# levje/TrackToLearn

Hardware: AMD Instinct MI355X
Metric: streamline-steps/s at n_actor=262144 (higher is better)
Workload: dtype f32

## Files before the change

include/ttl_hip.h:

```cpp
#ifndef TTL_HIP_H
#define TTL_HIP_H

#include <stddef.h>
#include <stdint.h>

#ifdef __cplusplus
extern "C" {
#endif

#if defined(__GNUC__) || defined(__clang__)
#define TTL_API __attribute__((visibility("default")))
#else
#define TTL_API
#endif

#define TTL_ABI_VERSION 13

#define TTL_OK 0
#define TTL_ERR_INVALID (-1)
#define TTL_ERR_HIP (-2)
#define TTL_ERR_STATE (-3)
#define TTL_ERR_UNSUPPORTED (-4)

#define TTL_MODE_F32 0
// ... 97 lines not shown

TTL_API int ttl_env_harvest_wait(ttl_env *env, const float *state_in, float *state_out,
                         int64_t state_pitch, void *hip_stream,
                         int32_t *n_continue_out);

TTL_API int ttl_env_freerun_begin(ttl_env *env, int32_t *host_counts, void *hip_stream);
TTL_API int ttl_env_freerun_step(ttl_env *env, const float *actions, int32_t n_rows,
                         float *state_out, int64_t state_pitch, double *reward_out,
                         uint8_t *done_out, void *hip_stream);
TTL_API int ttl_env_freerun_end(ttl_env *env, int32_t *n_active_out, int32_t *length_out,
                        int32_t *steps_out, void *hip_stream);
TTL_API int ttl_env_freerun_scripted_actions(ttl_env *env, const float *state, int64_t state_pitch,
                                     int32_t dir_offset, int32_t n_rows, uint32_t seed,
                                     float wobble, float *actions_out, void *hip_stream);

TTL_API int ttl_env_stopping_flags(ttl_env *env, const float *tail, int32_t n,
                           int32_t n_points, uint8_t *flags_out,
                           void *hip_stream);

TTL_API int ttl_env_set_processing_order(ttl_env *env, const int32_t *order, int32_t n,
                                 void *hip_stream);

TTL_API int ttl_env_refresh_processing_order(ttl_env *env, void *hip_stream);

TTL_API int ttl_env_view(ttl_env *env, const int32_t **continue_idx,
                 const int32_t **row_dest, int32_t *length);

#define TTL_PROFILE_CLASSES 4
TTL_API int ttl_env_profile_begin(ttl_env *env, int32_t max_launches,
                          int32_t class_mask );
TTL_API int ttl_env_profile_end(ttl_env *env, double *total_ms ,
                        int32_t *n_launches );

TTL_API int ttl_scripted_actions(const float *state, int64_t state_pitch,
                         int32_t dir_offset, const int32_t *continue_idx,
                         int32_t n, uint32_t seed, uint32_t step, float wobble,
                         float *actions_out, void *hip_stream);

TTL_API int ttl_peaks_from_sh(const float *sh, int64_t n_voxels, int32_t n_coef,
                      const float *sf_matrix, const float *vertices,
                      const int32_t *neighbours, int32_t n_vertices, int32_t degree,
                      int32_t npeaks, float relative_threshold, float absolute_threshold,
                      float min_separation_cos, int32_t max_candidates, float *peaks_out,
                      void *hip_stream);

TTL_API int ttl_oracle_net_forward(const float *dirs, int64_t n, const void *packed_half,
// ... 51 lines not shown
```

tracktolearn_amd/_lib.py:

```python
import ctypes as C
import os

import torch

_PKG = os.path.dirname(os.path.abspath(__file__))
LIB_PATH = os.path.join(_PKG, 'libttl_hip.so')

ABI_VERSION = 13
SH_LINEAR, SH_BRICK4 = 0, 1
MODE_F32 = 0
MODE_F64DIR = 1
MODE_F32NORM = 2
ORDER_ACTIVE = 0
ORDER_PARTITION = 1
ORDER_BY_POSITION = C.c_void_p(1)
ERR_INVALID, ERR_HIP, ERR_STATE, ERR_UNSUPPORTED = -1, -2, -3, -4


class TTLError(RuntimeError):
    pass


class EnvDesc(C.Structure):
    _fields_ = [
# ... 74 lines not shown
                                             C.c_void_p, C.c_void_p]),
    'ttl_tract_coverage': (C.c_int, [C.c_void_p, C.c_void_p, C.c_int32, C.c_void_p, C.c_float,
                                     C.POINTER(C.c_int32), C.c_void_p, C.c_void_p]),
    'ttl_oracle_bonus': (C.c_int, [C.c_void_p, C.c_int32, C.c_void_p, C.c_int32, C.c_double,
                                   C.c_int32, C.c_void_p, C.c_void_p, C.c_void_p]),
    'ttl_env_harvest_wait': (C.c_int, [C.c_void_p, C.c_void_p, C.c_void_p, C.c_int64,
                                       C.c_void_p, C.POINTER(C.c_int32)]),
    'ttl_env_harvest': (C.c_int, [C.c_void_p, C.c_void_p, C.c_void_p,
                                  C.c_int64, C.c_void_p]),
    'ttl_env_freerun_begin': (C.c_int, [C.c_void_p, C.c_void_p, C.c_void_p]),
    'ttl_env_freerun_step': (C.c_int, [C.c_void_p, C.c_void_p, C.c_int32, C.c_void_p,
                                       C.c_int64, C.c_void_p, C.c_void_p, C.c_void_p]),
    'ttl_env_freerun_scripted_actions': (C.c_int, [C.c_void_p, C.c_void_p, C.c_int64,
                                                   C.c_int32, C.c_int32, C.c_uint32,
                                                   C.c_float, C.c_void_p, C.c_void_p]),
    'ttl_env_freerun_end': (C.c_int, [C.c_void_p, C.POINTER(C.c_int32),
                                      C.POINTER(C.c_int32), C.POINTER(C.c_int32),
                                      C.c_void_p]),
    'ttl_env_stopping_flags': (C.c_int, [C.c_void_p, C.c_void_p, C.c_int32,
                                         C.c_int32, C.c_void_p, C.c_void_p]),
    'ttl_env_set_processing_order': (C.c_int, [C.c_void_p, C.c_void_p, C.c_int32,
                                               C.c_void_p]),
    'ttl_env_refresh_processing_order': (C.c_int, [C.c_void_p, C.c_void_p]),
    'ttl_env_view': (C.c_int, [C.c_void_p, C.POINTER(C.c_void_p),
                               C.POINTER(C.c_void_p), C.POINTER(C.c_int32)]),
    'ttl_env_profile_begin': (C.c_int, [C.c_void_p, C.c_int32, C.c_int32]),
    'ttl_env_profile_end': (C.c_int, [C.c_void_p, C.POINTER(C.c_double),
                                      C.POINTER(C.c_int32)]),
    'ttl_scripted_actions': (C.c_int, [C.c_void_p, C.c_int64, C.c_int32,
                                       C.c_void_p, C.c_int32, C.c_uint32,
                                       C.c_uint32, C.c_float, C.c_void_p,
                                       C.c_void_p]),
    'ttl_peaks_from_sh': (C.c_int, [C.c_void_p, C.c_int64, C.c_int32, C.c_void_p,
                                    C.c_void_p, C.c_void_p, C.c_int32, C.c_int32,
                                    C.c_int32, C.c_float, C.c_float, C.c_float,
                                    C.c_int32, C.c_void_p, C.c_void_p]),
    'ttl_resample_streamlines': (C.c_int, [C.c_void_p, C.c_int64, C.c_void_p,
                                           C.c_void_p, C.c_int32, C.c_int32,
                                           C.c_int32, C.c_void_p, C.c_void_p]),
    'ttl_oracle_net_forward': (C.c_int, [C.c_void_p, C.c_int64, C.c_void_p, C.c_void_p,
                                         C.c_void_p, C.c_void_p, C.c_void_p, C.c_void_p,
                                         C.c_int32, C.c_int32, C.c_int32, C.c_void_p,
                                         C.c_void_p]),
    'ttl_pack_streamlines': (C.c_int, [C.c_void_p, C.c_int64, C.c_void_p, C.c_void_p,
                                       C.c_int32, C.c_void_p, C.c_void_p]),
    'ttl_tract_mask_words': (C.c_int32, [C.c_int64]),
# ... 107 lines not shown
```

tracktolearn_amd/csrc/ttl_hip.hip:

```cpp
#include <hip/hip_runtime.h>

#include <atomic>
#include <chrono>
#include <cmath>
#include <cstdarg>
#include <cstdio>
#include <cstdlib>
#include <cstring>
#include <new>

#include "ttl_hip.h"

#include "ttl_internal.h"

#include <map>
#include <mutex>

namespace {
thread_local char g_err[512] = "";
}

int ttl_detail_fail(int code, const char *fmt, ...) {
    va_list ap;
    va_start(ap, fmt);
// ... 521 lines not shown
    if (active) rank = s_rank[threadIdx.x];
    if (active) {
        const size_t o = (size_t)blockIdx.x * BLOCK + rank;
        *reinterpret_cast<float4 *>(P.slot_head + 4 * o) = hd;
        P.slot_dest[o] = pd.y;
    }
    if (active) s_pos[rank] = pd.x;
    __syncthreads();
    const int pos = s_pos[threadIdx.x];
    const bool keep = pos >= 0;
    const unsigned long long mk = __ballot(keep);
    const int below = __popcll(mk & ((1ull << lane) - 1ull));
    if (lane == 0) red[wave] = __popcll(mk);
    __syncthreads();
    int wave_before = 0;
#pragma unroll
    for (int w = 0; w < BLOCK / 64; ++w)
        if (w < wave) wave_before += red[w];
    if (keep) proc_next[before + wave_before + below] = pos;
}

constexpr int TTL_TAIL_MAX_BLOCKS = 4096;

__global__ __launch_bounds__(BLOCK) void k_tail(
    EnvParams P, const int *__restrict__ idx, int *__restrict__ idx_next,
    const int *__restrict__ proc, int *__restrict__ proc_next, int n_active, int n_slots,
    int nb_rows, int order, int n_pts, int *__restrict__ host_word, int seq, int local_sort) {
    __shared__ int s_scan[TTL_TAIL_MAX_BLOCKS];
    __shared__ int s_wave[BLOCK / 64];
    __shared__ unsigned s_key[BLOCK];
    __shared__ int s_pos[BLOCK];
    __shared__ int s_rank[BLOCK];
    const int tid = threadIdx.x, lane = tid & 63, wave = tid >> 6;
    const int per = (nb_rows + BLOCK - 1) / BLOCK;
    const int lo = tid * per;
    int sum = 0;
    for (int k = 0; k < per; ++k)
        if (lo + k < nb_rows) sum += P.block_counts[lo + k];
    int incl = sum;
#pragma unroll
    for (int off = 1; off < 64; off <<= 1) {
        const int v = __shfl_up(incl, off);
        if (lane >= off) incl += v;
    }
    if (lane == 63) s_wave[wave] = incl;
    __syncthreads();
    int run = incl - sum, total = 0;
#pragma unroll
    for (int w = 0; w < BLOCK / 64; ++w) {
        if (w < wave) run += s_wave[w];
        total += s_wave[w];
    }
    for (int k = 0; k < per; ++k)
        if (lo + k < nb_rows) {
            s_scan[lo + k] = run;
// ... 25 lines not shown
    }
    const int j = i;
    const int row = j < n_slots ? proc[j] : -1;
    const bool live = row >= 0;
    float4 hd = float4{0.f, 0.f, 0.f, 0.f};
    int dest = -1, next = -1;
    if (live) {
        const bool stop = P.stop[row] != 0;
        const int pos = s_scan[row / BLOCK] + P.rank[row];
        dest = row;
        if (order == TTL_ORDER_PARTITION) dest = stop ? total + (row - pos) : pos;
        next = stop ? -1 : pos;
        hd = *reinterpret_cast<const float4 *>(P.head + 4 * (size_t)row);
    }
    if (!local_sort) {
        if (j < n_slots) {
            *reinterpret_cast<float4 *>(P.slot_head + 4 * (size_t)j) = hd;
            P.slot_dest[j] = dest;
            proc_next[j] = next;
        }
        return;
    }
    unsigned key = 0xFFFFFFFFu;
    if (live) {
        const unsigned vx = (unsigned)(int)fminf(fmaxf(floorf(hd.x), 0.0f), 1023.0f);
        const unsigned vy = (unsigned)(int)fminf(fmaxf(floorf(hd.y), 0.0f), 1023.0f);
        const unsigned vz = (unsigned)(int)fminf(fmaxf(floorf(hd.z), 0.0f), 1023.0f);
        const unsigned coarse = (((vx >> 6) & 3u) << 4) | (((vy >> 6) & 3u) << 2) | ((vz >> 6) & 3u);
        const unsigned m = (spread3(vx) << 2) | (spread3(vy) << 1) | spread3(vz);
        key = (min(coarse << 18 | m, 0xFFFFFEu) << 8) | (unsigned)tid;
    }
    unsigned sk = key;
#pragma unroll
    for (int size = 2; size <= 64; size <<= 1) {
#pragma unroll
        for (int stride = size >> 1; stride > 0; stride >>= 1) {
            const unsigned other = (unsigned)__shfl_xor((int)sk, stride);
            const bool up = (lane & size) == 0;
            const bool low = (lane & stride) == 0;
            const unsigned mn = min(sk, other), mx = max(sk, other);
            sk = (up == low) ? mn : mx;
        }
    }
    s_key[tid] = sk;
    s_pos[tid] = -1;
    const int n_live = __syncthreads_count(live);
    int srank = lane;
#pragma unroll
    for (int w = 0; w < BLOCK / 64; ++w) {
        if (w == wave) continue;
        const unsigned *srun = s_key + 64 * w;
        int c = 0;
#pragma unroll
        for (int step = 32; step > 0; step >>= 1)
            if (srun[c + step - 1] < sk) c += step;
        if (c == 63 && srun[63] < sk) c = 64;
        srank += c;
    }
    if (sk != 0xFFFFFFFFu) s_rank[sk & 255u] = srank;
    __syncthreads();
    const size_t base = (size_t)blockIdx.x * BLOCK;
    if (live) {
        const int rank = s_rank[tid];
        *reinterpret_cast<float4 *>(P.slot_head + 4 * (base + rank)) = hd;
        P.slot_dest[base + rank] = dest;
        s_pos[rank] = next;
    }
    __syncthreads();
    if (j < n_slots) {
        if (tid >= n_live) P.slot_dest[j] = -1;
        proc_next[j] = s_pos[tid];
    }
}

__global__ __launch_bounds__(BLOCK) void k_probe_flags(
    EnvParams P, const float *__restrict__ tail, int n, int n_pts,
    uint8_t *__restrict__ out) {
    const int i = blockIdx.x * BLOCK + threadIdx.x;
    if (i >= n) return;
    const float *t = tail + (size_t)i * 9;
    float ux, uy, uz, wx, wy, wz;
    int bits;
    if (n_pts >= 2) {
        bits = stopping_bits(P, t[0], t[1], t[2], t[3], t[4], t[5], t[6], t[7],
                             t[8], n_pts, ux, uy, uz, wx, wy, wz);
    } else {
        bits = (n_pts >= P.max_nb_steps) ? TTL_FLAG_LENGTH : 0;
        if (outside_mask(P, t[6], t[7], t[8])) bits |= TTL_FLAG_MASK;
    }
    out[i] = (uint8_t)bits;
}

__global__ __launch_bounds__(BLOCK) void k_finish(EnvParams P,
                                                  const int *__restrict__ idx,
                                                  int n_active, int n_pts) {
// ... 171 lines not shown

inline size_t align_up(size_t v, size_t a) { return (v + a - 1) / a * a; }

}

struct ttl_env {
    ttl_env_desc d;
    EnvParams P;
    int length;
    int n_active;
    int cur;
    int stepped;
    int last_order;
    int last_n;
    uint8_t *last_done;
    int *proc[2];
    char *order_ws;
    size_t order_ws_bytes;
    int proc_cur;
    int use_proc;
    int n_slots;
    int tail_fused;
    int tail_fused_max;
    int state_kernel;
    hipStream_t side;
    hipEvent_t ev_prefix;
    hipEvent_t ev_counts;
    int counts_pending;
    const int32_t *host_counts;
    const int32_t *host_probe;
    int *host_dev;
    int poll_seq;
    hipStream_t poll_stream;
    int fuse_small;
    int poll_counts;
    int local_sort;
    int n_exact;
    int fr_cap;
    int *fr_host_word;
    int prof_on;
    int prof_mask;
    int prof_cap;
    int prof_n[TTL_PROFILE_CLASSES];
    hipEvent_t *prof_ev[TTL_PROFILE_CLASSES];
};

// ... 16 lines not shown
    if (stop) e->prof_n[which]++;
}

extern "C" {

const char *ttl_last_error(void) { return g_err; }
uint32_t ttl_abi_version(void) { return TTL_ABI_VERSION; }
size_t ttl_env_desc_size(void) { return sizeof(ttl_env_desc); }

size_t ttl_env_workspace_bytes(int32_t n_max) {
    if (n_max < 0) return 0;
    const size_t n = (size_t)n_max;
    const size_t nb = (n + BLOCK - 1) / BLOCK + 1;
    size_t b = 0;
    b += align_up(n, 256);
    b += 6 * align_up(n * sizeof(int), 256);
    b += 2 * align_up(n * 4 * sizeof(float), 256);
    b += align_up(n * 8 * sizeof(float), 256);
    b += 2 * align_up(n * 2 * sizeof(int), 256);
    b += align_up(n * sizeof(int), 256);
    b += 2 * align_up(nb * sizeof(int), 256);
    b += 256;
    b += ttl_detail_order_workspace_bytes(n);
    return b;
}

int64_t ttl_sh_volume_records(const int32_t *dim, int32_t layout) {
    if (!dim || dim[0] < 1 || dim[1] < 1 || dim[2] < 1) return 0;
    if (layout == TTL_SH_BRICK4)
        return (int64_t)((dim[0] + 3) / 4) * ((dim[1] + 3) / 4) * ((dim[2] + 3) / 4) * 64;
    return (int64_t)dim[0] * dim[1] * dim[2];
}

struct VmmBlock {
    hipMemGenericAllocationHandle_t handle;
    size_t size;
};
static std::mutex g_vmm_mutex;
static std::map<void *, VmmBlock> g_vmm_blocks;

static hipError_t vmm_alloc(int device, size_t bytes, void **out) {
    hipMemAllocationProp prop{};
    prop.type = hipMemAllocationTypePinned;
    prop.location.type = hipMemLocationTypeDevice;
    prop.location.id = device;
    size_t gran = 0;
// ... 195 lines not shown
    P.lengths = d.lengths;
    P.dones = d.dones;
    const size_t n = (size_t)d.n_max;
    const size_t nb = (n + BLOCK - 1) / BLOCK + 1;
    char *w = (char *)d.workspace;
    P.stop = (uint8_t *)w;        w += align_up(n, 256);
    P.rank = (int *)w;            w += align_up(n * sizeof(int), 256);
    P.surv_pos = (int *)w;        w += align_up(n * sizeof(int), 256);
    P.row_dest = (int *)w;        w += align_up(n * sizeof(int), 256);
    P.block_counts = (int *)w;    w += align_up(nb * sizeof(int), 256);
    P.proc_rank = (int *)w;       w += align_up(n * sizeof(int), 256);
    P.proc_counts = (int *)w;     w += align_up(nb * sizeof(int), 256);
    e->proc[0] = (int *)w;        w += align_up(n * sizeof(int), 256);
    e->proc[1] = (int *)w;        w += align_up(n * sizeof(int), 256);
    P.head = (float *)w;          w += align_up(n * 4 * sizeof(float), 256);
    P.slot_head = (float *)w;     w += align_up(n * 4 * sizeof(float), 256);
    P.last2 = (float *)w;         w += align_up(n * 8 * sizeof(float), 256);
    P.pos_dest = (int *)w;        w += align_up(n * 2 * sizeof(int), 256);
    P.stop_list = (int *)w;       w += align_up(n * 2 * sizeof(int), 256);
    P.slot_dest = (int *)w;       w += align_up(n * sizeof(int), 256);
    P.counts = (int *)w;          w += 256;
    e->order_ws = w;
    e->order_ws_bytes = ttl_detail_order_workspace_bytes(n);
    e->length = 0;
    e->n_active = 0;
    e->cur = 0;
    e->stepped = 0;
    e->last_order = TTL_ORDER_ACTIVE;
    e->last_n = 0;
    e->last_done = nullptr;
    e->proc_cur = 0;
    e->use_proc = 0;
    e->state_kernel = 4;
    if (const char *v = getenv("TTL_STATE_KERNEL")) e->state_kernel = atoi(v);
    P.slot_rec = e->state_kernel != 2;
    P.xcd_remap = 1;
    if (const char *v = getenv("TTL_XCD_REMAP")) P.xcd_remap = atoi(v);
    P.xcd_rot = 0;
    if (const char *v = getenv("TTL_XCD_ROTATE")) P.xcd_rot = atoi(v) & 7;
    P.store_flavour = 0;
    if (const char *v = getenv("TTL_STORE_FLAVOUR")) P.store_flavour = atoi(v);
    e->side = nullptr;
    e->ev_prefix = nullptr;
    e->ev_counts = nullptr;
    e->counts_pending = 0;
    e->host_counts = nullptr;
// ... 113 lines not shown
        return fail(TTL_ERR_INVALID, "ttl_env_reset: null argument");
    const ttl_env_desc &d = env->d;
    if (n < 1 || n > d.n_max)
        return fail(TTL_ERR_INVALID, "ttl_env_reset: n=%d outside [1, %d]", n, d.n_max);
    const int64_t width = 7LL * d.n_coef + 3LL * d.n_dirs;
    if (state_pitch < width)
        return fail(TTL_ERR_INVALID, "ttl_env_reset: state_pitch %lld < %lld",
                    (long long)state_pitch, (long long)width);
    hipStream_t s = (hipStream_t)hip_stream;
    const size_t hist_bytes = (size_t)n * (size_t)(d.max_nb_steps + 1) * 3 * sizeof(float);
    HIP_TRY(hipMemsetAsync(d.streamlines, 0, hist_bytes, s));
    hipLaunchKernelGGL(k_reset, dim3((n + BLOCK - 1) / BLOCK), dim3(BLOCK), 0, s,
                       env->P, d.idx_a, seeds, n);
    HIP_TRY(hipGetLastError());
    env->cur = 0;
    env->length = 1;
    env->n_active = n;
    env->n_exact = 1;
    env->stepped = 0;
    env->fr_cap = 0;
    env->proc_cur = 0;
    env->use_proc = processing_order != nullptr;
    env->n_slots = n;
    if (processing_order == TTL_ORDER_BY_POSITION) {
        const int rc = ttl_detail_refresh_order(env->P, d.idx_a, n, env->order_ws,
                                                env->order_ws_bytes, env->proc[0], s);
        if (rc != TTL_OK) return rc;
    } else if (env->use_proc) {
        HIP_TRY(hipMemcpyAsync(env->proc[0], processing_order, (size_t)n * sizeof(int32_t),
                               hipMemcpyDeviceToDevice, s));
    }
    log_gather_rows(n);
    return ttl_detail_launch_state(env->P, env->state_kernel, nullptr, nullptr,
                                   env->use_proc ? env->proc[0] : nullptr, n, 1, state_out,
                                   state_pitch, s);
}

static hipError_t ttl_copy_counts(ttl_env *env, int32_t *host_counts, hipStream_t s) {
    hipError_t e;
    if (!env->side) {
        if ((e = hipStreamCreateWithFlags(&env->side, hipStreamNonBlocking)) != hipSuccess) return e;
        if ((e = hipEventCreateWithFlags(&env->ev_prefix, hipEventDisableTiming)) != hipSuccess) return e;
        if ((e = hipEventCreateWithFlags(&env->ev_counts, hipEventDisableTiming)) != hipSuccess) return e;
    }
    if ((e = hipEventRecord(env->ev_prefix, s)) != hipSuccess) return e;
    if ((e = hipStreamWaitEvent(env->side, env->ev_prefix, 0)) != hipSuccess) return e;
// ... 23 lines not shown
    if (noise && d.mode != TTL_MODE_F64DIR)
        return fail(TTL_ERR_INVALID, "ttl_env_step: noise needs TTL_MODE_F64DIR");
    hipStream_t s = (hipStream_t)hip_stream;
    const int *idx = env->cur ? d.idx_b : d.idx_a;
    const int L = env->length;
    const int nb = (n_active + BLOCK - 1) / BLOCK;
    prof_mark(env, 0, 0, s);
#define TTL_LAUNCH_ADVANCE(M)                                                  \
    hipLaunchKernelGGL((k_advance<M>), dim3(nb), dim3(BLOCK), 0, s, env->P, idx, \
                       actions, noise, n_active, L, reward_out, done_out)
    if (d.mode == TTL_MODE_F32) TTL_LAUNCH_ADVANCE(TTL_MODE_F32);
    else if (d.mode == TTL_MODE_F64DIR) TTL_LAUNCH_ADVANCE(TTL_MODE_F64DIR);
    else TTL_LAUNCH_ADVANCE(TTL_MODE_F32NORM);
#undef TTL_LAUNCH_ADVANCE
    prof_mark(env, 0, 1, s);
    HIP_TRY(hipGetLastError());
    env->length = L + 1;
    env->stepped = 2;
    env->last_n = n_active;
    env->last_done = done_out;
    return TTL_OK;
}

int ttl_env_step_end(ttl_env *env, const uint8_t *extra_flags, int32_t order,
                     float *state_out, int64_t state_pitch, int32_t *host_counts,
                     void *hip_stream) {
    if (!env || !state_out)
        return fail(TTL_ERR_INVALID, "ttl_env_step: null argument");
    if (env->stepped != 2)
        return fail(TTL_ERR_STATE, "ttl_env_step_end: call ttl_env_step_begin first");
    if (order != TTL_ORDER_ACTIVE && order != TTL_ORDER_PARTITION)
        return fail(TTL_ERR_INVALID, "ttl_env_step: bad order %d", order);
    const ttl_env_desc &d = env->d;
    const int64_t width = 7LL * d.n_coef + 3LL * d.n_dirs;
    if (state_pitch < width)
        return fail(TTL_ERR_INVALID, "ttl_env_step: state_pitch too small");
    hipStream_t s = (hipStream_t)hip_stream;
    const int *idx = env->cur ? d.idx_b : d.idx_a;
    int *idx_next = env->cur ? d.idx_a : d.idx_b;
    const int n_active = env->last_n;
    const int n_pts = env->length;
    const int nb = (n_active + BLOCK - 1) / BLOCK;
    if (extra_flags) {
        hipLaunchKernelGGL(k_restop, dim3(nb), dim3(BLOCK), 0, s, env->P, idx,
                           extra_flags, n_active, env->last_done);
        HIP_TRY(hipGetLastError());
    }
    if (env->use_proc && (n_active < 8192 ||
                          (env->fuse_small && ttl_detail_can_fuse_tail(env->P, n_active))))
        env->use_proc = 0;
    const int *proc = env->use_proc ? env->proc[env->proc_cur] : nullptr;
    env->stepped = 1;
    env->last_order = order;
    int *host_word = nullptr;
    int seq = 0;
    if (host_counts && env->poll_counts) {
        if (env->host_probe != host_counts) {
            void *dev = nullptr;
            env->host_probe = host_counts;
            env->host_dev = nullptr;
            if (hipHostGetDevicePointer(&dev, host_counts, 0) == hipSuccess)
                env->host_dev = static_cast<int *>(dev);
            else
                (void)hipGetLastError();
        }
        host_word = env->host_dev;
        static std::atomic<unsigned> g_seq{1};
        seq = (int)((g_seq.fetch_add(1, std::memory_order_relaxed) & 0x3fffffffu) | 0x40000000u);
    }
    if (host_word) {
        env->counts_pending = 2;
        env->host_counts = host_counts;
        env->poll_seq = seq;
        env->poll_stream = s;
    }
    if (!proc && env->fuse_small && env->state_kernel != 0 &&
        ttl_detail_can_fuse_tail(env->P, n_active)) {
        prof_mark(env, 2, 0, s);
        const int rc = ttl_detail_launch_fused_tail(env->P, idx, idx_next, n_active, order,
                                                    n_pts, state_out, state_pitch,
                                                    host_word, seq, s);
        prof_mark(env, 2, 1, s);
        if (rc != TTL_OK) return rc;
        if (host_counts && !host_word) HIP_TRY(ttl_copy_counts(env, host_counts, s));
        return TTL_OK;
    }
    int n_gather = n_active;
    const bool fused_tail = proc && env->tail_fused && env->P.slot_rec &&
                            ttl_detail_state_dedupes(env->P, env->state_kernel) &&
                            (env->n_slots < 0 ? n_active : env->n_slots) <= env->tail_fused_max;
    if (fused_tail) {
        if (env->n_slots < 0) env->n_slots = n_active;
        const int nbs = (env->n_slots + BLOCK - 1) / BLOCK;
        prof_mark(env, 1, 0, s);
        hipLaunchKernelGGL(k_tail, dim3(nbs), dim3(BLOCK), 0, s, env->P, idx, idx_next, proc,
                           env->proc[env->proc_cur ^ 1], n_active, env->n_slots, nb, order,
                           n_pts, host_word, seq, env->local_sort);
        prof_mark(env, 1, 1, s);
        HIP_TRY(hipGetLastError());
        if (host_counts && !host_word) HIP_TRY(ttl_copy_counts(env, host_counts, s));
        n_gather = env->n_slots;
    } else {
        if (proc && env->n_slots > n_active)
            return fail(TTL_ERR_STATE, "ttl_env_step: the processing order holds %d holes but "
                                       "the step tail was switched to the two-kernel form; "
                                       "refresh the order first", env->n_slots - n_active);
        prof_mark(env, 1, 0, s);
        hipLaunchKernelGGL(k_prefix, dim3(nb), dim3(BLOCK), 0, s, env->P, idx, idx_next,
                           proc, n_active, nb, order, n_pts, host_word, seq);
        prof_mark(env, 1, 1, s);
        HIP_TRY(hipGetLastError());
        if (host_counts && !host_word) {
            HIP_TRY(ttl_copy_counts(env, host_counts, s));
        }
        if (proc) {
            prof_mark(env, 3, 0, s);
            hipLaunchKernelGGL(k_proc_scatter, dim3(nb), dim3(BLOCK), 0, s, env->P, idx, proc,
                               env->proc[env->proc_cur ^ 1], n_active, nb,
                               env->local_sort && env->P.slot_rec);
            prof_mark(env, 3, 1, s);
            HIP_TRY(hipGetLastError());
            env->n_slots = -1;
        }
    }
    prof_mark(env, 2, 0, s);
    log_gather_rows(n_active);
    const int rc = ttl_detail_launch_state(env->P, env->state_kernel, idx, env->P.row_dest,
                                           proc, n_gather, n_pts, state_out, state_pitch, s);
    prof_mark(env, 2, 1, s);
    return rc;
}

int ttl_env_step(ttl_env *env, const float *actions, const double *noise,
                 int32_t n_active, int32_t order, float *state_out,
                 int64_t state_pitch, double *reward_out, uint8_t *done_out,
                 int32_t *host_counts, void *hip_stream) {
    if (!state_out) return fail(TTL_ERR_INVALID, "ttl_env_step: null argument");
    if (order != TTL_ORDER_ACTIVE && order != TTL_ORDER_PARTITION)
        return fail(TTL_ERR_INVALID, "ttl_env_step: bad order %d", order);
    if (env) {
        const int64_t width = 7LL * env->d.n_coef + 3LL * env->d.n_dirs;
        if (state_pitch < width)
            return fail(TTL_ERR_INVALID, "ttl_env_step: state_pitch too small");
    }
    const int rc = ttl_env_step_begin(env, actions, noise, n_active, reward_out,
                                      done_out, hip_stream);
    if (rc != TTL_OK) return rc;
    return ttl_env_step_end(env, nullptr, order, state_out, state_pitch,
                            host_counts, hip_stream);
}

int ttl_env_harvest(ttl_env *env, const float *state_in, float *state_out,
// ... 198 lines not shown
        return fail(TTL_ERR_INVALID, "ttl_env_stopping_flags: n and n_points must be >= 1");
    hipLaunchKernelGGL(k_probe_flags, dim3((n + BLOCK - 1) / BLOCK), dim3(BLOCK), 0,
                       (hipStream_t)hip_stream, env->P, tail, n, n_points,
                       flags_out);
    HIP_TRY(hipGetLastError());
    return TTL_OK;
}

int ttl_env_set_processing_order(ttl_env *env, const int32_t *order, int32_t n,
                                 void *hip_stream) {
    if (!env || !order) return fail(TTL_ERR_INVALID, "ttl_env_set_processing_order: null argument");
    if (env->length < 1 || env->stepped)
        return fail(TTL_ERR_STATE, "ttl_env_set_processing_order: between harvest and step only");
    if (!env->n_exact || n != env->n_active)
        return fail(TTL_ERR_INVALID, "ttl_env_set_processing_order: n=%d, %d rows are active",
                    n, env->n_active);
    HIP_TRY(hipMemcpyAsync(env->proc[env->proc_cur], order, (size_t)n * sizeof(int32_t),
                           hipMemcpyDeviceToDevice, (hipStream_t)hip_stream));
    env->use_proc = 1;
    env->n_slots = n;
    return TTL_OK;
}

int ttl_env_refresh_processing_order(ttl_env *env, void *hip_stream) {
    if (!env) return fail(TTL_ERR_INVALID, "ttl_env_refresh_processing_order: null handle");
    if (env->length < 1 || env->stepped)
        return fail(TTL_ERR_STATE, "ttl_env_refresh_processing_order: between harvest and step only");
    if (!env->n_exact)
        return fail(TTL_ERR_STATE, "ttl_env_refresh_processing_order: survivor count not read back yet");
    const int *idx = env->cur ? env->d.idx_b : env->d.idx_a;
    const int rc = ttl_detail_refresh_order(env->P, idx, env->n_active, env->order_ws,
                                            env->order_ws_bytes, env->proc[env->proc_cur],
                                            (hipStream_t)hip_stream);
    if (rc == TTL_OK) {
        env->use_proc = 1;
        env->n_slots = env->n_active;
    }
    return rc;
}

int ttl_pack_streamlines(const float *history, int64_t row_pitch, const int64_t *keep,
                         const int64_t *offsets, int32_t n, float *points_out,
                         void *hip_stream) {
    if (!history || !keep || !offsets || !points_out || n < 1 || row_pitch < 3)
        return fail(TTL_ERR_INVALID, "ttl_pack_streamlines: bad arguments");
    const int per_block = BLOCK / 64;
// ... 18 lines not shown
```

tracktolearn_amd/csrc/ttl_internal.h:

```cpp
#ifndef TTL_INTERNAL_H
#define TTL_INTERNAL_H
#include <hip/hip_runtime.h>

#include <cstdint>

#include "ttl_hip.h"

int ttl_detail_fail(int code, const char *fmt, ...) __attribute__((format(printf, 2, 3)));
#define fail ttl_detail_fail

#define HIP_TRY(expr)                                                        \
    do {                                                                     \
        hipError_t e_ = (expr);                                              \
        if (e_ != hipSuccess)                                                \
            return fail(TTL_ERR_HIP, "%s: %s", #expr, hipGetErrorString(e_)); \
    } while (0)

constexpr int TTL_BLOCK = 256;

struct EnvParams {
    int mode;
    int sh_dim[3];
    int n_coef;
    int coef_pitch;
// ... 59 lines not shown
    return P.sh_brick ? (unsigned)(z >> 2) * 64u + (unsigned)(z & 3) : (unsigned)z;
}

inline size_t ttl_detail_sh_records(const EnvParams &P) {
    if (!P.sh_brick) return (size_t)P.sh_dim[0] * P.sh_dim[1] * P.sh_dim[2];
    return (size_t)((P.sh_dim[0] + 3) / 4) * ((P.sh_dim[1] + 3) / 4) *
           ((P.sh_dim[2] + 3) / 4) * 64;
}

int ttl_detail_launch_state(const EnvParams &P, int state_kernel, const int *idx,
                            const int *row_dest, const int *proc, int n_rows, int L,
                            float *out, int64_t pitch, hipStream_t s);
bool ttl_detail_state_dedupes(const EnvParams &P, int state_kernel);
bool ttl_detail_can_fuse_tail(const EnvParams &P, int n_active);
int ttl_detail_launch_fused_tail(const EnvParams &P, const int *idx, int *idx_next,
                                 int n_active, int order, int n_pts, float *out,
                                 int64_t pitch, int *host_word, int seq, hipStream_t s);
int ttl_detail_launch_fused_tail_fr(const EnvParams &P, int *idx_a, int *idx_b, int n_cap,
                                    float *out, int64_t pitch, int *host_word,
                                    hipStream_t s);
size_t ttl_detail_order_workspace_bytes(size_t n);
int ttl_detail_refresh_order(const EnvParams &P, const int *idx, int n, char *ws,
                             size_t ws_bytes, int *order_out, hipStream_t s);
#endif
```

tracktolearn_amd/csrc/ttl_order.hip:

```cpp
#include "ttl_internal.h"

#include <cstdlib>
#include <cstring>

#include <rocprim/device/device_radix_sort.hpp>

namespace {
constexpr int BLOCK = TTL_BLOCK;

__global__ __launch_bounds__(BLOCK) void k_order_keys(const float *__restrict__ last2,
                                                      const int *__restrict__ idx, int n,
                                                      int nbx, int nby, int nbz, int fine,
                                                      unsigned *__restrict__ keys,
                                                      int *__restrict__ rows) {
    const int i = blockIdx.x * BLOCK + threadIdx.x;
    if (i >= n) return;
    const float *p = last2 + 8 * (size_t)idx[i] + 4;
    const int nb[3] = {nbx, nby, nbz};
    unsigned b[3], m = 0;
#pragma unroll
    for (int a = 0; a < 3; ++a) {
        const float vox = floorf(p[a] + 0.5f);
        const float v = floorf(vox * 0.125f);
        b[a] = (unsigned)fminf(fmaxf(v == v ? v : 0.0f, 0.0f), (float)(nb[a] - 1));
// ... 74 lines not shown
    unsigned key[SORT_ITEMS], rank[SORT_ITEMS];
#pragma unroll
    for (int k = 0; k < SORT_ITEMS; ++k) {
        const int i = base + k * BLOCK + threadIdx.x;
        key[k] = 0;
        rank[k] = 0;
        if (i < n) {
            key[k] = keys[i];
            rank[k] = atomicAdd(&s_bin[key[k]], 1u);
        }
    }
    __syncthreads();
    for (int b = threadIdx.x; b < bins; b += BLOCK) {
        const unsigned c = s_bin[b];
        if (c) s_bin[b] = atomicAdd(&gcursor[b], c);
    }
    __syncthreads();
#pragma unroll
    for (int k = 0; k < SORT_ITEMS; ++k) {
        const int i = base + k * BLOCK + threadIdx.x;
        if (i < n) out[s_bin[key[k]] + rank[k]] = rows[i];
    }
}
}

size_t ttl_detail_order_workspace_bytes(size_t n) {
    return 3 * ((n * 4 + 255) / 256 * 256) + (4u << 20) + n * 24;
}

int ttl_detail_refresh_order(const EnvParams &P, const int *idx, int n, char *ws,
                             size_t ws_bytes, int *order_out, hipStream_t s) {
    const size_t slab = ((size_t)n * 4 + 255) / 256 * 256;
    if (ws_bytes < 3 * slab) return fail(TTL_ERR_INVALID, "order refresh: workspace too small");
    unsigned *keys_in = reinterpret_cast<unsigned *>(ws);
    unsigned *keys_out = reinterpret_cast<unsigned *>(ws + slab);
    int *rows_in = reinterpret_cast<int *>(ws + 2 * slab);
    void *temp = ws + 3 * slab;
    const size_t temp_avail = ws_bytes - 3 * slab;
    int nb[3];
    unsigned long long bricks = 1;
    for (int a = 0; a < 3; ++a) {
        nb[a] = (P.sh_dim[a] + 7) / 8 + 1;
        if (nb[a] > 1024) nb[a] = 1024;
        bricks *= (unsigned long long)nb[a];
    }
    unsigned bits = 1;
// ... 43 lines not shown
```

tracktolearn_amd/environments/tracking_env.py:

```python
import ctypes as C
import os
import time

import numpy as np
import torch

from tracktolearn_amd import _lib
from tracktolearn_amd.environments.env import BaseEnv
from tracktolearn_amd.environments.stopping_criteria import StoppingFlags
from tracktolearn_amd.tractogram import Tractogram


class _StepInfo(dict):

    def __init__(self, env, n_active, reward_info):
        super().__init__(reward_info=reward_info)
        self._env, self._n = env, n_active
        self._idx_dev = env._idx_view(n_active)

    def __missing__(self, key):
        if key == 'continue_idx':
            val = self._idx_dev.to('cpu').numpy().astype(np.int64)
            self[key] = val
            return val
# ... 143 lines not shown
        _lib.check(self._lib.ttl_env_reset(
            self._handle, seeds32.data_ptr(), n,
            _lib.ORDER_BY_POSITION if sort_rows else None, state.data_ptr(),
            self._state_pitch, self._stream()), 'ttl_env_reset')
        self._n_total = n
        self._n_active = n
        self._order_slots = n if sort_rows else 0
        self._cur = 0
        self.length = 1
        self._pending = None
        self.not_stopping = None
        return state

    SPATIAL_ORDER_MIN = min(max(int(os.environ.get('TTL_FUSE_MAX_ROWS', '16384')), 256), 65536)

    SPATIAL_ORDER_REFRESH = int(os.environ.get('TTL_ORDER_REFRESH', '16'))

    def _refresh_processing_order(self, force=False):
        every = self.SPATIAL_ORDER_REFRESH
        n = self._n_active
        if n < self.SPATIAL_ORDER_MIN or self._pending is not None or \
                not getattr(self, 'spatial_order', True):
            return
        slots = getattr(self, '_order_slots', 0)
        sparse = bool(every) and self.length > 1 and slots and n < self.ORDER_MIN_FILL * slots \
            and slots <= self.TAIL_FUSED_MAX_ROWS and self._order_keeps_holes()
        if not force and not sparse and \
                (not every or self.length <= 1 or (self.length - 1) % every):
            return
        _lib.check(self._lib.ttl_env_refresh_processing_order(
            self._handle, self._stream()), 'ttl_env_refresh_processing_order')
        self._order_slots = n

    def _order_keeps_holes(self):
        return os.environ.get('TTL_STATE_KERNEL', '') not in ('0', '2') and \
            bool(self.add_neighborhood_vox) and \
            0.0 < float(np.float32(self.add_neighborhood_vox)) < 1.0

    ORDER_MIN_FILL = float(os.environ.get('TTL_ORDER_MIN_FILL', '0.8'))
    TAIL_FUSED_MAX_ROWS = 0 if os.environ.get('TTL_TAIL_FUSED', '1') == '0' else \
        min(int(os.environ.get('TTL_TAIL_FUSED_MAX_ROWS', '262144')), 4096 * 256)

    def nreset(self, n_seeds: int):
        replace = n_seeds > len(self.seeds)
        picks = np.random.choice(
            np.arange(len(self.seeds)), size=n_seeds, replace=replace)
        return self._start(self.seeds[picks])

    def reset(self, start: int, end: int):
        return self._start(self.seeds[start:end])

    def _host_io(self):
        if self._io is None:
            n = self._n_max
            io = dict(
# ... 463 lines not shown
```

Measured before the change: 783.5 million.

## Rebucket processing order inside fused tail kernel instead of periodic radix sort

Extends the fused tail kernel to compute a coarse 8-voxel brick bin per live row and atomically reserve per-bin offsets. A new scatter kernel then rebuilds the spatial processing order from these records every few steps. The Python side skips the separate periodic radix-sort refresh when this in-step mode is active, removing a sort and its extra launches in exchange for atomics and a coarser spatial ordering.

```diff
diff --git a/include/ttl_hip.h b/include/ttl_hip.h
--- a/include/ttl_hip.h
+++ b/include/ttl_hip.h
@@ -143,6 +143,8 @@
                                  void *hip_stream);
 
 TTL_API int ttl_env_refresh_processing_order(ttl_env *env, void *hip_stream);
+
+TTL_API int ttl_env_order_slots(ttl_env *env, int32_t *n_slots_out, int32_t *instep_out);
 
 TTL_API int ttl_env_view(ttl_env *env, const int32_t **continue_idx,
                  const int32_t **row_dest, int32_t *length);
diff --git a/tracktolearn_amd/_lib.py b/tracktolearn_amd/_lib.py
--- a/tracktolearn_amd/_lib.py
+++ b/tracktolearn_amd/_lib.py
@@ -120,6 +120,7 @@
     'ttl_env_set_processing_order': (C.c_int, [C.c_void_p, C.c_void_p, C.c_int32,
                                                C.c_void_p]),
     'ttl_env_refresh_processing_order': (C.c_int, [C.c_void_p, C.c_void_p]),
+    'ttl_env_order_slots': (C.c_int, [C.c_void_p, C.POINTER(C.c_int32), C.POINTER(C.c_int32)]),
     'ttl_env_view': (C.c_int, [C.c_void_p, C.POINTER(C.c_void_p),
                                C.POINTER(C.c_void_p), C.POINTER(C.c_int32)]),
     'ttl_env_profile_begin': (C.c_int, [C.c_void_p, C.c_int32, C.c_int32]),
diff --git a/tracktolearn_amd/csrc/ttl_hip.hip b/tracktolearn_amd/csrc/ttl_hip.hip
--- a/tracktolearn_amd/csrc/ttl_hip.hip
+++ b/tracktolearn_amd/csrc/ttl_hip.hip
@@ -567,15 +567,19 @@
 
 constexpr int TTL_TAIL_MAX_BLOCKS = 4096;
 
+template <bool REBUCKET>
 __global__ __launch_bounds__(BLOCK) void k_tail(
     EnvParams P, const int *__restrict__ idx, int *__restrict__ idx_next,
     const int *__restrict__ proc, int *__restrict__ proc_next, int n_active, int n_slots,
-    int nb_rows, int order, int n_pts, int *__restrict__ host_word, int seq, int local_sort) {
+    int nb_rows, int order, int n_pts, int *__restrict__ host_word, int seq, int local_sort,
+    int2 *__restrict__ ord_rec, unsigned *__restrict__ bin_count, int nbx, int nby, int nbz) {
     __shared__ int s_scan[TTL_TAIL_MAX_BLOCKS];
     __shared__ int s_wave[BLOCK / 64];
     __shared__ unsigned s_key[BLOCK];
     __shared__ int s_pos[BLOCK];
     __shared__ int s_rank[BLOCK];
+    __shared__ int s_bin[REBUCKET ? BLOCK : 1];
+    __shared__ unsigned long long s_heads[BLOCK / 64];
     const int tid = threadIdx.x, lane = tid & 63, wave = tid >> 6;
     const int per = (nb_rows + BLOCK - 1) / BLOCK;
     const int lo = tid * per;
@@ -647,6 +651,7 @@
         return;
     }
     unsigned key = 0xFFFFFFFFu;
+    int bin = -1;
     if (live) {
         const unsigned vx = (unsigned)(int)fminf(fmaxf(floorf(hd.x), 0.0f), 1023.0f);
         const unsigned vy = (unsigned)(int)fminf(fmaxf(floorf(hd.y), 0.0f), 1023.0f);
@@ -654,6 +659,9 @@
         const unsigned coarse = (((vx >> 6) & 3u) << 4) | (((vy >> 6) & 3u) << 2) | ((vz >> 6) & 3u);
         const unsigned m = (spread3(vx) << 2) | (spread3(vy) << 1) | spread3(vz);
         key = (min(coarse << 18 | m, 0xFFFFFEu) << 8) | (unsigned)tid;
+        if (REBUCKET && next >= 0)
+            bin = (min((int)(vx >> 3), nbx - 1) * nby + min((int)(vy >> 3), nby - 1)) * nbz +
+                  min((int)(vz >> 3), nbz - 1);
     }
     unsigned sk = key;
 #pragma unroll
@@ -669,6 +677,7 @@
     }
     s_key[tid] = sk;
     s_pos[tid] = -1;
+    if (REBUCKET) s_bin[tid] = -1;
     const int n_live = __syncthreads_count(live);
     int srank = lane;
 #pragma unroll
@@ -690,12 +699,34 @@
         *reinterpret_cast<float4 *>(P.slot_head + 4 * (base + rank)) = hd;
         P.slot_dest[base + rank] = dest;
         s_pos[rank] = next;
+        if (REBUCKET) s_bin[rank] = bin;
     }
     __syncthreads();
-    if (j < n_slots) {
-        if (tid >= n_live) P.slot_dest[j] = -1;
-        proc_next[j] = s_pos[tid];
-    }
+    if (j < n_slots && tid >= n_live) P.slot_dest[j] = -1;
+    if (!REBUCKET) {
+        if (j < n_slots) proc_next[j] = s_pos[tid];
+        return;
+    }
+    const int b = s_bin[tid];
+    const bool head = tid == 0 || s_bin[tid - 1] != b;
+    const bool last = tid == BLOCK - 1 || s_bin[tid + 1] != b;
+    const unsigned long long hm = __ballot(head);
+    if (lane == 0) s_heads[wave] = hm;
+    __syncthreads();
+    int hp = 0;
+    for (int w = wave; w >= 0; --w) {
+        unsigned long long mk = s_heads[w];
+        if (w == wave) mk &= (2ull << lane) - 1ull;
+        if (mk) {
+            hp = 64 * w + 63 - __clzll(mk);
+            break;
+        }
+    }
+    if (last && b >= 0) s_rank[hp] = (int)atomicAdd(&bin_count[b], (unsigned)(tid - hp + 1));
+    __syncthreads();
+    if (j < n_slots)
+        ord_rec[j] = int2{b >= 0 ? (int)(((unsigned)b << TTL_INSTEP_OFF_BITS) | (unsigned)(s_rank[hp] + (tid - hp))) : -1,
+                          s_pos[tid]};
 }
 
 __global__ __launch_bounds__(BLOCK) void k_probe_flags(
@@ -913,6 +944,14 @@
     int n_slots;
     int tail_fused;
     int tail_fused_max;
+    int proc_min_rows;
+    int instep;
+    int instep_after;
+    int instep_bins;
+    int instep_nb[3];
+    int2 *ord_rec;
+    unsigned *ord_count[2];
+    int ord_parity;
     int state_kernel;
     hipStream_t side;
     hipEvent_t ev_prefix;
@@ -975,6 +1014,8 @@
     b += 2 * align_up(nb * sizeof(int), 256);
     b += 256;
     b += ttl_detail_order_workspace_bytes(n);
+    b += align_up(n * sizeof(int2), 256);
+    b += 2 * align_up(ttl_detail_order_instep_count_bytes(), 256);
     return b;
 }
 
@@ -1216,6 +1257,20 @@
     P.counts = (int *)w;          w += 256;
     e->order_ws = w;
     e->order_ws_bytes = ttl_detail_order_workspace_bytes(n);
+    w += e->order_ws_bytes;
+    e->ord_rec = (int2 *)w;       w += align_up(n * sizeof(int2), 256);
+    for (int k = 0; k < 2; ++k) {
+        e->ord_count[k] = (unsigned *)w;
+        w += align_up(ttl_detail_order_instep_count_bytes(), 256);
+    }
+    e->ord_parity = 0;
+    e->proc_min_rows = 8192;
+    if (const char *v = getenv("TTL_ORDER_MIN_ROWS")) e->proc_min_rows = atoi(v);
+    e->instep = 2;
+    if (const char *v = getenv("TTL_ORDER_INSTEP")) e->instep = atoi(v) > 0 ? atoi(v) : 0;
+    e->instep_after = 0;
+    if (const char *v = getenv("TTL_ORDER_INSTEP_AFTER")) e->instep_after = atoi(v) != 0;
+    e->instep_bins = ttl_detail_order_bins(P, e->instep_nb);
     e->length = 0;
     e->n_active = 0;
     e->cur = 0;
@@ -1375,6 +1430,12 @@
     env->proc_cur = 0;
     env->use_proc = processing_order != nullptr;
     env->n_slots = n;
+    if (env->instep && env->instep_bins) {
+        HIP_TRY(hipMemsetAsync(env->ord_count[0], 0,
+                               (size_t)((char *)env->ord_count[1] - (char *)env->ord_count[0]) +
+                                   ttl_detail_order_instep_count_bytes(), s));
+        env->ord_parity = 0;
+    }
     if (processing_order == TTL_ORDER_BY_POSITION) {
         const int rc = ttl_detail_refresh_order(env->P, d.idx_a, n, env->order_ws,
                                                 env->order_ws_bytes, env->proc[0], s);
@@ -1444,6 +1505,23 @@
     return TTL_OK;
 }
 
+static bool ttl_order_instep_on(const ttl_env *env, int slots) {
+    return env->instep > 0 && env->instep_bins > 0 && env->local_sort && env->tail_fused &&
+           env->P.slot_rec && ttl_detail_state_dedupes(env->P, env->state_kernel) &&
+           slots <= env->tail_fused_max && slots <= (1 << TTL_INSTEP_OFF_BITS);
+}
+
+static int ttl_order_instep_scatter(ttl_env *env, hipStream_t s) {
+    const int rc = ttl_detail_order_scatter(env->ord_rec, env->n_slots,
+                                            env->ord_count[env->ord_parity],
+                                            env->ord_count[env->ord_parity ^ 1], env->instep_bins,
+                                            env->proc[env->proc_cur ^ 1], s);
+    if (rc != TTL_OK) return rc;
+    env->ord_parity ^= 1;
+    env->n_slots = -1;
+    return TTL_OK;
+}
+
 int ttl_env_step_end(ttl_env *env, const uint8_t *extra_flags, int32_t order,
                      float *state_out, int64_t state_pitch, int32_t *host_counts,
                      void *hip_stream) {
@@ -1468,7 +1546,7 @@
                            extra_flags, n_active, env->last_done);
         HIP_TRY(hipGetLastError());
     }
-    if (env->use_proc && (n_active < 8192 ||
+    if (env->use_proc && (n_active < env->proc_min_rows ||
                           (env->fuse_small && ttl_detail_can_fuse_tail(env->P, n_active))))
         env->use_proc = 0;
     const int *proc = env->use_proc ? env->proc[env->proc_cur] : nullptr;
@@ -1508,6 +1586,7 @@
         return TTL_OK;
     }
     int n_gather = n_active;
+    bool rebucket = false;
     const bool fused_tail = proc && env->tail_fused && env->P.slot_rec &&
                             ttl_detail_state_dedupes(env->P, env->state_kernel) &&
                             (env->n_slots < 0 ? n_active : env->n_slots) <= env->tail_fused_max;
@@ -1515,13 +1594,26 @@
         if (env->n_slots < 0) env->n_slots = n_active;
         const int nbs = (env->n_slots + BLOCK - 1) / BLOCK;
         prof_mark(env, 1, 0, s);
-        hipLaunchKernelGGL(k_tail, dim3(nbs), dim3(BLOCK), 0, s, env->P, idx, idx_next, proc,
-                           env->proc[env->proc_cur ^ 1], n_active, env->n_slots, nb, order,
-                           n_pts, host_word, seq, env->local_sort);
+        rebucket = ttl_order_instep_on(env, env->n_slots) && (n_pts - 1) % env->instep == 0;
+        unsigned *cnt = env->ord_count[env->ord_parity];
+        if (rebucket)
+            hipLaunchKernelGGL(k_tail<true>, dim3(nbs), dim3(BLOCK), 0, s, env->P, idx, idx_next,
+                               proc, env->proc[env->proc_cur ^ 1], n_active, env->n_slots, nb,
+                               order, n_pts, host_word, seq, env->local_sort, env->ord_rec, cnt,
+                               env->instep_nb[0], env->instep_nb[1], env->instep_nb[2]);
+        else
+            hipLaunchKernelGGL(k_tail<false>, dim3(nbs), dim3(BLOCK), 0, s, env->P, idx, idx_next,
+                               proc, env->proc[env->proc_cur ^ 1], n_active, env->n_slots, nb,
+                               order, n_pts, host_word, seq, env->local_sort, nullptr, nullptr,
+                               0, 0, 0);
         prof_mark(env, 1, 1, s);
         HIP_TRY(hipGetLastError());
         if (host_counts && !host_word) HIP_TRY(ttl_copy_counts(env, host_counts, s));
         n_gather = env->n_slots;
+        if (rebucket && !env->instep_after) {
+            const int rc = ttl_order_instep_scatter(env, s);
+            if (rc != TTL_OK) return rc;
+        }
     } else {
         if (proc && env->n_slots > n_active)
             return fail(TTL_ERR_STATE, "ttl_env_step: the processing order holds %d holes but "
@@ -1550,6 +1642,7 @@
     const int rc = ttl_detail_launch_state(env->P, env->state_kernel, idx, env->P.row_dest,
                                            proc, n_gather, n_pts, state_out, state_pitch, s);
     prof_mark(env, 2, 1, s);
+    if (rc == TTL_OK && rebucket && env->instep_after) return ttl_order_instep_scatter(env, s);
     return rc;
 }
 
@@ -1794,6 +1887,15 @@
     return TTL_OK;
 }
 
+int ttl_env_order_slots(ttl_env *env, int32_t *n_slots_out, int32_t *instep_out) {
+    if (!env || !n_slots_out)
+        return fail(TTL_ERR_INVALID, "ttl_env_order_slots: null argument");
+    const int slots = !env->use_proc ? 0 : env->n_slots < 0 ? env->n_active : env->n_slots;
+    *n_slots_out = slots;
+    if (instep_out) *instep_out = ttl_order_instep_on(env, slots) ? env->instep : 0;
+    return TTL_OK;
+}
+
 int ttl_env_refresh_processing_order(ttl_env *env, void *hip_stream) {
     if (!env) return fail(TTL_ERR_INVALID, "ttl_env_refresh_processing_order: null handle");
     if (env->length < 1 || env->stepped)
diff --git a/tracktolearn_amd/csrc/ttl_internal.h b/tracktolearn_amd/csrc/ttl_internal.h
--- a/tracktolearn_amd/csrc/ttl_internal.h
+++ b/tracktolearn_amd/csrc/ttl_internal.h
@@ -105,4 +105,9 @@
 size_t ttl_detail_order_workspace_bytes(size_t n);
 int ttl_detail_refresh_order(const EnvParams &P, const int *idx, int n, char *ws,
                              size_t ws_bytes, int *order_out, hipStream_t s);
+int ttl_detail_order_bins(const EnvParams &P, int nb[3]);
+size_t ttl_detail_order_instep_count_bytes();
+constexpr int TTL_INSTEP_OFF_BITS = 18;
+int ttl_detail_order_scatter(const int2 *rec, int n_slots, const unsigned *count,
+                             unsigned *count_other, int bins, int *order_out, hipStream_t s);
 #endif
diff --git a/tracktolearn_amd/csrc/ttl_order.hip b/tracktolearn_amd/csrc/ttl_order.hip
--- a/tracktolearn_amd/csrc/ttl_order.hip
+++ b/tracktolearn_amd/csrc/ttl_order.hip
@@ -120,6 +120,88 @@
         if (i < n) out[s_bin[key[k]] + rank[k]] = rows[i];
     }
 }
+constexpr int INSTEP_MAX_BINS = SORT_MAX_BINS - BLOCK / 64;
+constexpr int INSTEP_ITEMS = 4;
+
+__global__ __launch_bounds__(BLOCK) void k_order_scatter(const int2 *__restrict__ rec, int n_slots,
+                                                         const unsigned *__restrict__ gcount,
+                                                         unsigned *__restrict__ gcount_other,
+                                                         int bins, int *__restrict__ out) {
+    extern __shared__ unsigned s_bin[];
+    unsigned *s_wave = s_bin + bins;
+    const int tid = threadIdx.x, lane = tid & 63, wave = tid >> 6;
+    const int base = blockIdx.x * (BLOCK * INSTEP_ITEMS) + tid;
+    int2 r[INSTEP_ITEMS];
+#pragma unroll
+    for (int k = 0; k < INSTEP_ITEMS; ++k) {
+        const int j = base + k * BLOCK;
+        r[k] = j < n_slots ? rec[j] : int2{-1, -1};
+    }
+    for (int b = tid; b < bins; b += BLOCK) s_bin[b] = gcount[b];
+    for (int b = blockIdx.x * BLOCK + tid; b < bins; b += gridDim.x * BLOCK) gcount_other[b] = 0;
+    __syncthreads();
+    const int per = (bins + BLOCK - 1) / BLOCK;
+    const int lo = tid * per;
+    unsigned sum = 0;
+    for (int k = 0; k < per; ++k)
+        if (lo + k < bins) sum += s_bin[lo + k];
+    unsigned incl = sum;
+#pragma unroll
+    for (int off = 1; off < 64; off <<= 1) {
+        const unsigned v = __shfl_up(incl, off);
+        if (lane >= off) incl += v;
+    }
+    if (lane == 63) s_wave[wave] = incl;
+    __syncthreads();
+    unsigned run = incl - sum, total = 0;
+#pragma unroll
+    for (int w = 0; w < BLOCK / 64; ++w) {
+        if (w < wave) run += s_wave[w];
+        total += s_wave[w];
+    }
+    for (int k = 0; k < per; ++k)
+        if (lo + k < bins) {
+            const unsigned c = s_bin[lo + k];
+            s_bin[lo + k] = run;
+            run += c;
+        }
+    __syncthreads();
+#pragma unroll
+    for (int k = 0; k < INSTEP_ITEMS; ++k) {
+        const int j = base + k * BLOCK;
+        if (j >= n_slots) continue;
+        if ((unsigned)j >= total) out[j] = -1;
+        if (r[k].x != -1) {
+            const unsigned p = s_bin[(unsigned)r[k].x >> TTL_INSTEP_OFF_BITS] +
+                               ((unsigned)r[k].x & ((1u << TTL_INSTEP_OFF_BITS) - 1u));
+            if (p < (unsigned)n_slots) out[p] = r[k].y;
+        }
+    }
+}
+}
+
+int ttl_detail_order_bins(const EnvParams &P, int nb[3]) {
+    unsigned long long bricks = 1;
+    for (int a = 0; a < 3; ++a) {
+        nb[a] = (P.sh_dim[a] + 7) / 8 + 1;
+        if (nb[a] > 1024) nb[a] = 1024;
+        bricks *= (unsigned long long)nb[a];
+    }
+    return bricks <= (unsigned long long)INSTEP_MAX_BINS ? (int)bricks : 0;
+}
+
+size_t ttl_detail_order_instep_count_bytes() { return (size_t)SORT_MAX_BINS * sizeof(unsigned); }
+
+int ttl_detail_order_scatter(const int2 *rec, int n_slots, const unsigned *count,
+                             unsigned *count_other, int bins, int *order_out, hipStream_t s) {
+    if (bins < 1 || bins > INSTEP_MAX_BINS || n_slots < 1 || n_slots > (1 << TTL_INSTEP_OFF_BITS))
+        return fail(TTL_ERR_INVALID, "order scatter: %d bins, %d slots", bins, n_slots);
+    const size_t lds = ((size_t)bins + BLOCK / 64) * sizeof(unsigned);
+    const int chunk = BLOCK * INSTEP_ITEMS;
+    hipLaunchKernelGGL(k_order_scatter, dim3((n_slots + chunk - 1) / chunk), dim3(BLOCK), lds, s,
+                       rec, n_slots, count, count_other, bins, order_out);
+    HIP_TRY(hipGetLastError());
+    return TTL_OK;
 }
 
 size_t ttl_detail_order_workspace_bytes(size_t n) {
diff --git a/tracktolearn_amd/environments/tracking_env.py b/tracktolearn_amd/environments/tracking_env.py
--- a/tracktolearn_amd/environments/tracking_env.py
+++ b/tracktolearn_amd/environments/tracking_env.py
@@ -189,6 +189,8 @@
         if n < self.SPATIAL_ORDER_MIN or self._pending is not None or \
                 not getattr(self, 'spatial_order', True):
             return
+        if not force and self._order_instep():
+            return
         slots = getattr(self, '_order_slots', 0)
         sparse = bool(every) and self.length > 1 and slots and n < self.ORDER_MIN_FILL * slots \
             and slots <= self.TAIL_FUSED_MAX_ROWS and self._order_keeps_holes()
@@ -198,6 +200,14 @@
         _lib.check(self._lib.ttl_env_refresh_processing_order(
             self._handle, self._stream()), 'ttl_env_refresh_processing_order')
         self._order_slots = n
+
+    def _order_instep(self):
+        slots, period = C.c_int32(0), C.c_int32(0)
+        _lib.check(self._lib.ttl_env_order_slots(
+            self._handle, C.byref(slots), C.byref(period)), 'ttl_env_order_slots')
+        if period.value:
+            self._order_slots = slots.value
+        return period.value
 
     def _order_keeps_holes(self):
         return os.environ.get('TTL_STATE_KERNEL', '') not in ('0', '2') and \
```

Result: faster. 804.0 million (median of 6 runs) (+2.6%).
